# stardist/stardist

Hardware: AMD Instinct MI355X
Metric: predict_instances() Mpix/s (2D) + Mvox/s (3D) end-to-end at 1/2/4/8 GPU (higher is better)
Workload: dtype f32

## Files before the change

### include/stardist_hip.h

```cpp
#ifndef STARDIST_HIP_H
#define STARDIST_HIP_H

#include <stdbool.h>
#include <stdint.h>

#ifdef __cplusplus
extern "C" {
#endif

const char* sd_last_error(void);
int sd_version(void);
int sd_device_count(void);
int sd_release_workspace(void);
int sd_set_option(const char* name, int value);
int sd_get_option(const char* name);

int sd_nms2d_host(const float* dist, const float* points, int n_polys, int n_rays,
                  int use_kdtree, int use_bbox, int verbose, float threshold,
                  uint8_t* keep, int64_t* stats);
int sd_nms2d_device(const float* d_dist, const float* d_points, int n_polys, int n_rays,
                    int use_kdtree, int use_bbox, int verbose, float threshold,
                    uint8_t* d_keep, int64_t* stats, void* stream);

int sd_nms2d_old_host(const int32_t* polys, int n_polys, int n_rays, const int32_t* mapping, int height, int width,
                      float threshold, int max_bbox_search, int grid_y, int grid_x, int verbose, uint8_t* keep);
int sd_nms2d_old_device(const int32_t* d_polys, int n_polys, int n_rays, const int32_t* d_mapping, int height, int width,
                        float threshold, int max_bbox_search, int grid_y, int grid_x, int verbose, uint8_t* d_keep, void* stream);

int sd_prepare_polys_device(const int32_t* d_x, const int32_t* d_y, int n_polys, int n_verts, void* d_out,
                            int64_t out_bytes, void* stream);

int sd_clip_pairs_device(const int32_t* d_xa, const int32_t* d_ya, const int32_t* d_xb,
                         const int32_t* d_yb, int n_pairs, int n_verts,
                         int64_t* d_out_twice_area, int32_t* d_out_flags, void* stream);

int sd_area_bounds_pairs_device(const int32_t* d_xa, const int32_t* d_ya, const int32_t* d_xb, const int32_t* d_yb, int n_pairs,
                                int n_verts, float* d_out_area, float* d_out_band, int32_t* d_out_info, void* stream);

int sd_star_dist2d_host(const uint16_t* src, int H, int W, int n_rays, int grid_y, int grid_x,
                        float* dst);
int sd_star_dist2d_device(const uint16_t* d_src, int H, int W, int n_rays, int grid_y,
                          int grid_x, float* d_dst, void* stream);
int sd_star_dist3d_host(const uint16_t* src, int Z, int Y, int X, const float* dz,
                        const float* dy, const float* dx, int n_rays, int grid_z, int grid_y,
                        int grid_x, float* dst);
int sd_star_dist3d_device(const uint16_t* d_src, int Z, int Y, int X, const float* d_dz,
                          const float* d_dy, const float* d_dx, int n_rays, int grid_z,
                          int grid_y, int grid_x, float* d_dst, void* stream);

int sd_edt_prob_device(const int32_t* d_lbl, int Z, int Y, int X, double sz, double sy, double sx, int max_label,
                       float* d_prob, void* stream);

int sd_polygons_to_label_host(const float* coord, const int32_t* labels, int n_polys, int n_rays,
                              int H, int W, int32_t* result);
int sd_polygons_to_label_device(const float* d_coord, const int32_t* d_labels, int n_polys,
                                int n_rays, int H, int W, int32_t* d_result, void* stream);
int sd_polygons_to_label_window_device(const float* d_coord, const int32_t* d_labels, int n_polys, int n_rays, int HI, int WI,
                                       int y0, int x0, int H, int W, int32_t* d_result, void* stream);

int sd_dist_to_coord_device(const float* d_dist, const double* d_points, const double* d_sincos, long long n_polys, int n_rays,
// ... 157 lines not shown
```

### stardist_amd/csrc/area_bounds.h

```cpp
#pragma once
#include <hip/hip_runtime.h>

namespace sdarea {

enum { PP_PLAIN = 1, PP_POS = 2, PP_NEG = 4 };
struct PolyProps { float lmax, perim; int flags; int xmin, xmax, ymin, ymax; int pad; };

__device__ __forceinline__ float sgnf(float v) { return v > 0.f ? 1.f : (v < 0.f ? -1.f : 0.f); }
__device__ __forceinline__ float half_sum(float v) { for (int o = 16; o; o >>= 1) v += __shfl_xor(v, o); return v; }
__device__ __forceinline__ float half_max(float v) { for (int o = 16; o; o >>= 1) v = fmaxf(v, __shfl_xor(v, o)); return v; }
__device__ __forceinline__ int half_sum_i(int v) { for (int o = 16; o; o >>= 1) v += __shfl_xor(v, o); return v; }
__device__ __forceinline__ int half_min_i(int v) { for (int o = 16; o; o >>= 1) { const int t = __shfl_xor(v, o); v = t < v ? t : v; } return v; }
__device__ __forceinline__ int half_max_i(int v) { for (int o = 16; o; o >>= 1) { const int t = __shfl_xor(v, o); v = t > v ? t : v; } return v; }

constexpr float NEAR_W = 0.15f, STRIP_W = 0.45f;
constexpr int WINDOW = 2047;

static __global__ void __launch_bounds__(256) k_poly_props(const int* __restrict__ vx, const int* __restrict__ vy, int n, int R, PolyProps* __restrict__ out) {
  const int lane = threadIdx.x & 63, half = lane >> 5, l = lane & 31, hb = half << 5;
  const int wave = blockIdx.x * (blockDim.x >> 6) + (threadIdx.x >> 6);
  const int cand = 2 * wave + half;
  const bool cv = cand < n;
  const bool valid = cv && l < R;
  int X = 0, Y = 0;
  if (valid) { X = vx[(size_t)cand * R + l]; Y = vy[(size_t)cand * R + l]; }
  const int x0 = __shfl(X, hb), y0 = __shfl(Y, hb);
  const int xmin = half_min_i(valid ? X : 0x7fffffff), xmax = half_max_i(valid ? X : (int)0x80000000);
  const int ymin = half_min_i(valid ? Y : 0x7fffffff), ymax = half_max_i(valid ? Y : (int)0x80000000);
  const bool small = cv && (long long)xmax - xmin <= WINDOW && (long long)ymax - ymin <= WINDOW;
  const int ln = (l + 1 >= R) ? 0 : l + 1;
  const int rx = valid && small ? X - x0 : 0, ry = valid && small ? Y - y0 : 0;
  const int rbx = __shfl(rx, hb + ln), rby = __shfl(ry, hb + ln);
  const float ax = (float)rx, ay = (float)ry, bx = (float)rbx, by = (float)rby;
  const float ex = bx - ax, ey = by - ay;
  const bool deg = !valid || (ex == 0.f && ey == 0.f);
  const unsigned long long bal = __ballot(!deg);
  const unsigned int m32 = (unsigned int)(half ? (bal >> 32) : bal);
  const int count = __popc(m32);
  int nxt = -1;
  if (m32) { const unsigned int above = (l >= 31) ? 0u : (m32 & ~((2u << l) - 1u)); nxt = above ? __ffs((int)above) - 1 : __ffs((int)m32) - 1; }
  const int area2 = half_sum_i(valid ? rx * rby - ry * rbx : 0);
  bool bad = false;
  __shared__ float2 sv[4][2][32];
  __shared__ int sn[4][2][32];
  const int wv = threadIdx.x >> 6;
  sv[wv][half][l] = make_float2(ax, ay); sn[wv][half][l] = nxt;
  __builtin_amdgcn_wave_barrier();
  for (int dd = 1; dd <= (R >> 1); ++dd) {
    int k = l + dd; if (k >= R) k -= R;
    if (!valid) k = 0;
    const int kn = (k + 1 >= R) ? 0 : k + 1;
    const float2 c2 = sv[wv][half][k], d2 = sv[wv][half][kn];
    const float cx = c2.x, cy = c2.y, dx = d2.x, dy = d2.y;
    const int nxt_k = sn[wv][half][k];
    const bool degk = ((m32 >> k) & 1u) == 0u;
    const float fx = dx - cx, fy = dy - cy;
    if (valid && small && !degk && !((cx == ax && cy == ay) || (dx == ax && dy == ay)) && ay >= fminf(cy, dy) && ay <= fmaxf(cy, dy)) {
      if (fy == 0.f) { if (ax >= fminf(cx, dx) && ax <= fmaxf(cx, dx)) bad = true; }
      else if (2.f * fabsf((cx - ax) * fy + (ay - cy) * fx) <= fabsf(fy)) bad = true;
    }
    if (valid && small && !deg && !((ax == cx && ay == cy) || (bx == cx && by == cy)) && cy >= fminf(ay, by) && cy <= fmaxf(ay, by)) {
      if (ey == 0.f) { if (cx >= fminf(ax, bx) && cx <= fmaxf(ax, bx)) bad = true; }
      else if (2.f * fabsf((ax - cx) * ey + (cy - ay) * ex) <= fabsf(ey)) bad = true;
    }
    if (deg || degk || !valid) continue;
    if (k == nxt || nxt_k == l) {
      const float cr = ex * fy - ey * fx, dt = ex * fx + ey * fy;
      if (cr == 0.f && dt < 0.f) bad = true;
      continue;
    }
    const float o1 = ex * (cy - ay) - ey * (cx - ax), o2 = ex * (dy - ay) - ey * (dx - ax);
    const float o3 = fx * (ay - cy) - fy * (ax - cx), o4 = fx * (by - cy) - fy * (bx - cx);
    bool inter = (sgnf(o1) * sgnf(o2) <= 0.f) && (sgnf(o3) * sgnf(o4) <= 0.f);
    if (o1 == 0.f && o2 == 0.f)
      inter = fmaxf(fminf(ax, bx), fminf(cx, dx)) <= fminf(fmaxf(ax, bx), fmaxf(cx, dx)) &&
              fmaxf(fminf(ay, by), fminf(cy, dy)) <= fminf(fmaxf(ay, by), fmaxf(cy, dy));
    if (inter) bad = true;
  }
  const unsigned long long badm = __ballot(bad);
  const bool anybad = (unsigned int)(half ? (badm >> 32) : badm) != 0u;
  const float lmax = half_max(deg ? 0.f : sqrtf(ex * ex + ey * ey));
  const float perim = half_sum(deg ? 0.f : fabsf(ex) + fabsf(ey));
  if (cv && l == 0) {
    PolyProps p;
    p.lmax = lmax * (1.f + 1e-6f); p.perim = perim;
    p.flags = ((small && !anybad && count >= 3 && area2 != 0) ? PP_PLAIN : 0) | (area2 > 0 ? PP_POS : 0) | (area2 < 0 ? PP_NEG : 0);
    p.xmin = xmin; p.xmax = xmax; p.ymin = ymin; p.ymax = ymax; p.pad = 0;
    out[cand] = p;
  }
}

struct Enclosure { float area, band; int crossings, near; bool usable; };

__device__ __forceinline__ Enclosure pair_enclosure(const int* __restrict__ px, const int* __restrict__ py, const int* __restrict__ qx,
                                                    const int* __restrict__ qy, int R, const PolyProps& pp, const PolyProps& pq, bool active,
                                                    float2* sq, int l, int half) {
  Enclosure E; E.area = 0.f; E.band = 0.f; E.crossings = 0; E.near = 0; E.usable = false;
  const int hb = half << 5;
  bool use = active && (pp.flags & PP_PLAIN) && (pq.flags & PP_PLAIN) && ((pp.flags & (PP_POS | PP_NEG)) == (pq.flags & (PP_POS | PP_NEG)));
  const int ox = use ? (int)(((long long)pp.xmin + pp.xmax) >> 1) : 0, oy = use ? (int)(((long long)pp.ymin + pp.ymax) >> 1) : 0;
  long long ext = 0;
  if (use) {
    const long long e0 = (long long)pp.xmax - ox, e1 = (long long)ox - pp.xmin, e2 = (long long)pp.ymax - oy, e3 = (long long)oy - pp.ymin;
    const long long e4 = (long long)pq.xmax - ox, e5 = (long long)ox - pq.xmin, e6 = (long long)pq.ymax - oy, e7 = (long long)oy - pq.ymin;
    ext = e0; ext = e1 > ext ? e1 : ext; ext = e2 > ext ? e2 : ext; ext = e3 > ext ? e3 : ext;
    ext = e4 > ext ? e4 : ext; ext = e5 > ext ? e5 : ext; ext = e6 > ext ? e6 : ext; ext = e7 > ext ? e7 : ext;
    if (ext > WINDOW / 2) use = false;
  }
  const bool lv = use && l < R;
  float ax = 0.f, ay = 0.f, cqx = 0.f, cqy = 0.f;
  if (lv) { ax = (float)(px[l] - ox); ay = (float)(py[l] - oy); cqx = (float)(qx[l] - ox); cqy = (float)(qy[l] - oy); }
  sq[l] = make_float2(cqx, cqy);
  const int ln = (l + 1 >= R) ? 0 : l + 1;
// ... 83 lines not shown
```

### stardist_amd/csrc/area_bounds.hip

```cpp
#include "common.h"
#include "area_bounds.h"
#include "../../include/stardist_hip.h"

namespace {
__global__ void __launch_bounds__(256) k_area_probe(const int* __restrict__ xa, const int* __restrict__ ya, const int* __restrict__ xb,
                                                    const int* __restrict__ yb, int n, int R, const sdarea::PolyProps* __restrict__ pa,
                                                    const sdarea::PolyProps* __restrict__ pb, float* __restrict__ out_area, float* __restrict__ out_band,
                                                    int* __restrict__ out_info) {
  __shared__ float2 sq[4][2][32];
  const int lane = threadIdx.x & 63, half = lane >> 5, l = lane & 31, wv = threadIdx.x >> 6;
  const long long nw = (long long)gridDim.x * 4;
  for (long long base = 2ll * ((long long)blockIdx.x * 4 + wv); base < n; base += 2ll * nw) {
    const long long t = base + half;
    const bool active = t < n;
    const long long tt = active ? t : 0;
    const sdarea::Enclosure E = sdarea::pair_enclosure(xa + tt * R, ya + tt * R, xb + tt * R, yb + tt * R, R, pa[tt], pb[tt], active, sq[wv][half], l, half);
    if (active && l == 0) { out_area[t] = E.area; out_band[t] = E.band; out_info[t] = (E.usable ? 1 : 0) | ((E.crossings & 0x3FF) << 8) | ((E.near & 0x7FF) << 18); }
    __builtin_amdgcn_wave_barrier();
  }
}
}

extern "C" int sd_area_bounds_pairs_device(const int32_t* d_xa, const int32_t* d_ya, const int32_t* d_xb, const int32_t* d_yb, int n_pairs, int n_verts,
                                           float* d_out_area, float* d_out_band, int32_t* d_out_info, void* stream) {
  hipStream_t s = (hipStream_t)stream;
  if (n_pairs <= 0) return 0;
  const int R = n_verts;
  if (R < 3 || R > 32) { sd::set_error("sd_area_bounds_pairs: n_verts=%d unsupported (3..32)", R); return -1; }
  sd::Arena& A = sd::arena();
  if (A.begin(s)) return -1;
  sdarea::PolyProps* pa = (sdarea::PolyProps*)A.take((size_t)n_pairs * sizeof(sdarea::PolyProps));
  sdarea::PolyProps* pb = (sdarea::PolyProps*)A.take((size_t)n_pairs * sizeof(sdarea::PolyProps));
  if (!pa || !pb) return -1;
  hipLaunchKernelGGL(sdarea::k_poly_props, dim3(sd::div_up(n_pairs, 8)), dim3(256), 0, s, d_xa, d_ya, n_pairs, R, pa);
  hipLaunchKernelGGL(sdarea::k_poly_props, dim3(sd::div_up(n_pairs, 8)), dim3(256), 0, s, d_xb, d_yb, n_pairs, R, pb);
  const int blocks = sd::div_up(n_pairs, 8) < 2048 ? sd::div_up(n_pairs, 8) : 2048;
  hipLaunchKernelGGL(k_area_probe, dim3(blocks), dim3(256), 0, s, d_xa, d_ya, d_xb, d_yb, n_pairs, R, pa, pb, d_out_area, d_out_band, d_out_info);
  SD_LAUNCH_CHECK();
  SD_CHECK(hipStreamSynchronize(s));
  return 0;
}
```

### stardist_amd/csrc/nms2d.hip

```cpp
#include <type_traits>

#include "common.h"
#include "clip_sweep.h"
#include "clip_beam.h"
#include "area_bounds.h"
#include "../../include/stardist_hip.h"
#include <hipcub/hipcub.hpp>
#include <math.h>
#include <stdlib.h>
#include <vector>

namespace {

using sdclip::i64;

enum { ST_UNDECIDED = 0, ST_KEPT = 1, ST_SUPPRESSED = 2 };

__device__ __forceinline__ float wave_min(float v) { for (int o = 32; o; o >>= 1) v = fminf(v, __shfl_xor(v, o)); return v; }
__device__ __forceinline__ float wave_max(float v) { for (int o = 32; o; o >>= 1) v = fmaxf(v, __shfl_xor(v, o)); return v; }
__device__ __forceinline__ i64 wave_sum(i64 v) { for (int o = 32; o; o >>= 1) v += __shfl_xor(v, o); return v; }

__global__ void __launch_bounds__(256) k_build(const float* __restrict__ dist, const float* __restrict__ pts,
                                               const float2* __restrict__ sincos, int N, int R,
                                               int* __restrict__ vx, int* __restrict__ vy, int4* __restrict__ bbox,
                                               float* __restrict__ radius, float* __restrict__ area, int* gstats) {
  extern __shared__ int lds[];
  const int wave = threadIdx.x >> 6, lane = threadIdx.x & 63;
  const int i = blockIdx.x * (blockDim.x >> 6) + wave;
// ... 712 lines not shown
}

__global__ void k_count_after(unsigned int* out, const unsigned int* total, const unsigned int* first) { *out = *total > *first ? *total - *first : 0u; }
__global__ void k_iota(int* a, int n) { int i = blockIdx.x * blockDim.x + threadIdx.x; if (i < n) a[i] = i; }
__global__ void k_keep(const unsigned char* __restrict__ state, unsigned char* __restrict__ keep, int n) {
  int i = blockIdx.x * blockDim.x + threadIdx.x;
  if (i < n) keep[i] = (state[i] != ST_SUPPRESSED);
}

}

namespace sd {
int clip_full_pairs(const int2* d_pairs, const unsigned int* d_idx, const unsigned int* d_n, unsigned int cap, int R, const int* d_vx, const int* d_vy,
                    const float* d_area, float thr, unsigned char* d_state, unsigned char* d_supp, unsigned int* d_errCount, hipStream_t stream);
}

namespace {
struct Counters { int nU, nK, nS, left; unsigned long long nPairs; unsigned int nSpill, nExact, nErr, nDecided; };

template <int MAXV, int SPREP>
struct BeamPath {
  typedef sdclip::PolyPrep<MAXV> Prep;
  static int prepare(const int* vx, const int* vy, int N, int R, void* prep, hipStream_t s) {
    const size_t lds = sdclip::PrepWork<sdclip::LdsStorage<SPREP>, MAXV>::lds_bytes() + 64;
    hipLaunchKernelGGL((k_prepare<MAXV, SPREP>), dim3(sd::div_up(N, SPREP)), dim3(SPREP), lds, s, vx, vy, N, R, (Prep*)prep);
    SD_LAUNCH_CHECK();
    return 0;
  }
  static int tier1(const int2* pairs, const unsigned int* idx, const unsigned long long* nPairs, const unsigned int* first, const void* prep, const float* area,
                   float thr, unsigned char* state, unsigned char* supp, PairQueues q, hipStream_t s) {
    const int lanes = sd::option(sd::OPT_NMS2D_PAIR_LANES);
    if (lanes == 32) {
      static const size_t lds32 = beam_lds_bytes<MAXV, 8, 6, 4, 32>();
      hipLaunchKernelGGL((k_pairs_beam<MAXV, 8, 6, 4, 32, unsigned long long>), dim3(256 * 8), dim3(32), lds32, s, pairs, idx, nPairs, first, (const Prep*)prep, area, thr, state, supp, q);
    } else if (lanes == 6464) {
      static const size_t lds = beam_lds_bytes<MAXV, 8, 6, 4, 64>();
      hipLaunchKernelGGL((k_pairs_beam<MAXV, 8, 6, 4, 64, unsigned long long>), dim3(256 * 4), dim3(64), lds, s, pairs, idx, nPairs, first, (const Prep*)prep, area, thr, state, supp, q);
    } else {
      static const size_t lds16 = beam_lds_bytes<MAXV, 8, 6, 4, 64, true>();
      static const int per_cu = (int)((160 * 1024) / lds16);
      hipLaunchKernelGGL((k_pairs_beam<MAXV, 8, 6, 4, 64, unsigned long long, true>), dim3(256 * per_cu), dim3(64), lds16, s, pairs, idx, nPairs, first, (const Prep*)prep, area, thr, state, supp, q);
    }
    SD_LAUNCH_CHECK();
    return 0;
  }
  template <typename CNT>
  static int tier2(const int2* pairs, const unsigned int* idx, const CNT* nPairs, const unsigned int* first, const void* prep, const float* area, float thr,
                   unsigned char* state, unsigned char* supp, PairQueues q, hipStream_t s) {
    static const size_t lds = beam_lds_bytes<MAXV, 15, 16, 8, 32>();
    hipLaunchKernelGGL((k_pairs_beam<MAXV, 15, 16, 8, 32, CNT>), dim3(256 * 3), dim3(32), lds, s, pairs, idx, nPairs, first, (const Prep*)prep, area, thr, state, supp, q);
// ... 68 lines not shown
  if (R <= 32) prepStride = sizeof(sdclip::PolyPrep<32>); else if (R <= 64) prepStride = sizeof(sdclip::PolyPrep<64>);
  else if (R <= 128) prepStride = sizeof(sdclip::PolyPrep<128>); else prepStride = sizeof(sdclip::PolyPrep<256>);
  void* prep = A.take((size_t)N * prepStride);
  if (!prep) return -1;
  hipStream_t side = side_stream();
  if (!side) return -1;
  hipEvent_t evFork = nullptr, evJoin = nullptr;
  SD_CHECK(hipEventCreateWithFlags(&evFork, hipEventDisableTiming));
  SD_CHECK(hipEventCreateWithFlags(&evJoin, hipEventDisableTiming));
  EvGuard evguardFJ{evFork, evJoin};
  const bool areaBounds = R <= 32 && R >= 3 && sd::option(sd::OPT_NMS2D_AREA_BOUNDS) != 0 && sd::option(sd::OPT_NMS2D_STRICT) == 0;
  sdarea::PolyProps* props = nullptr;
  hipEvent_t evProps = nullptr, evPrep = nullptr;
  SD_CHECK(hipEventCreateWithFlags(&evProps, hipEventDisableTiming));
  SD_CHECK(hipEventCreateWithFlags(&evPrep, hipEventDisableTiming));
  EvGuard evguardP{evProps, evPrep};
  if (areaBounds) {
    props = (sdarea::PolyProps*)A.take((size_t)N * sizeof(sdarea::PolyProps));
    if (!props) return -1;
  }
  auto launch_side = [&]() -> int {
    SD_CHECK(hipEventRecord(evFork, s));
    SD_CHECK(hipStreamWaitEvent(side, evFork, 0));
    if (areaBounds) {
      hipLaunchKernelGGL(sdarea::k_poly_props, dim3(sd::div_up(N, 8)), dim3(256), 0, side, vx, vy, N, R, props);
      SD_LAUNCH_CHECK();
    }
    SD_CHECK(hipEventRecord(evProps, side));
    int rc;
    if (R <= 32) rc = BeamPath<32, 64>::prepare(vx, vy, N, R, prep, side);
    else if (R <= 64) rc = BeamPath<64, 64>::prepare(vx, vy, N, R, prep, side);
    else if (R <= 128) rc = BeamPath<128, 32>::prepare(vx, vy, N, R, prep, side);
    else rc = BeamPath<256, 16>::prepare(vx, vy, N, R, prep, side);
    if (rc) return -1;
    SD_CHECK(hipEventRecord(evPrep, side));
    SD_CHECK(hipEventRecord(evJoin, side));
    return 0;
  };
  int gs[8];
  SD_CHECK(hipMemcpyAsync(gs, gstats, sizeof(gs), hipMemcpyDeviceToHost, s));
  SD_CHECK(hipStreamSynchronize(s));
  float max_dist;
  memcpy(&max_dist, &gs[0], 4);

  GridP g;
  const float reach = (max_dist + 1.f) * 1.0001f + 1e-3f;
  const int by_bbox = (threshold >= 0.f || use_bbox) ? 1 : 0;
  float cs = 0.5f * reach;
  if (!(cs >= 1.f)) cs = 1.f;
  for (;;) {
    g.ny = (int)(((double)gs[2] - gs[1]) / cs) + 1;
    g.nx = (int)(((double)gs[4] - gs[3]) / cs) + 1;
    if ((long long)g.ny * g.nx <= (1ll << 26)) break;
    cs *= 2.f;
  }
  g.y0 = (float)gs[1]; g.x0 = (float)gs[3]; g.inv_cs = 1.f / cs;
  const int nCells = g.ny * g.nx;
// ... 501 lines not shown
```

### stardist_amd/csrc/nms2d_full.hip

```cpp
#include <type_traits>

#include "common.h"
#include "clip_sweep.h"
#include "clip_sweep_full.h"
#include "clip_beam.h"
#include <stdlib.h>
#include "../../include/stardist_hip.h"

namespace {
using sdclip::i64;

enum { ST_SUPPRESSED_ = 2 };
template <int MAXV, int MAXIL, int MAXREC, int MAXPT, int MAXJ>
__global__ void __launch_bounds__(64) k_full_pairs(const int2* __restrict__ pairs, const unsigned int* __restrict__ idx, const unsigned int* __restrict__ nPtr, unsigned int cap, int R,
                                                   const int* __restrict__ vx, const int* __restrict__ vy,
                                                   const float* __restrict__ area, float thr, unsigned char* __restrict__ state, unsigned char* __restrict__ supp,
                                                   unsigned int* errCount) {
  unsigned int n = *nPtr; if (n > cap) n = cap;
  for (unsigned int t = threadIdx.x * gridDim.x + blockIdx.x; t < n; t += gridDim.x * blockDim.x) {
    if (MAXV > 64 && __hip_atomic_load(errCount, __ATOMIC_RELAXED, __HIP_MEMORY_SCOPE_AGENT) != 0u) break;
    const unsigned int p = idx ? idx[t] : t;
    const int2 ij = pairs[p];
    sdclip::SweepFull<MAXV, MAXIL, MAXREC, MAXPT, MAXJ> sw;
    sw.reset_state();
    sw.add_path(vx + (size_t)ij.x * R, vy + (size_t)ij.x * R, R, sdclip::kClip, 0);
    sw.add_path(vx + (size_t)ij.y * R, vy + (size_t)ij.y * R, R, sdclip::kSubject, MAXV);
    const i64 twice = sw.execute();
    if (sw.status & ~sdclip::ST_FAIL) atomicAdd(errCount, 1u);
// ... 107 lines not shown
  if (R <= 32) {
    static const size_t ldsBytes = lds_full_bytes<32, 64, 32, 192, 64>();
    static bool attr_set = false;
    if (!attr_set) {
      SD_CHECK(hipFuncSetAttribute((const void*)k_full_pairs_lds<32, 64, 32, 192, 64>, hipFuncAttributeMaxDynamicSharedMemorySize, (int)ldsBytes));
      attr_set = true;
    }
    hipLaunchKernelGGL((k_full_pairs_lds<32, 64, 32, 192, 64>), dim3(1024), dim3(LDSF_T), ldsBytes, s, d_pairs, d_idx, d_n, cap, R, d_vx, d_vy, d_area, thr, d_state, d_supp, d_errCount);
  } else if (R <= 64) hipLaunchKernelGGL((k_full_pairs<64, 96, 48, 384, 96>), dim3(2048), dim3(64), 0, s, d_pairs, d_idx, d_n, cap, R, d_vx, d_vy, d_area, thr, d_state, d_supp, d_errCount);
  else if (R <= 128) hipLaunchKernelGGL((k_full_pairs<128, 128, 64, 768, 128>), dim3(512), dim3(64), 0, s, d_pairs, d_idx, d_n, cap, R, d_vx, d_vy, d_area, thr, d_state, d_supp, d_errCount);
  else hipLaunchKernelGGL((k_full_pairs<256, 192, 96, 1536, 192>), dim3(256), dim3(64), 0, s, d_pairs, d_idx, d_n, cap, R, d_vx, d_vy, d_area, thr, d_state, d_supp, d_errCount);
  SD_LAUNCH_CHECK();
  return 0;
}
}

extern "C" int sd_prepare_polys_device(const int32_t* d_x, const int32_t* d_y, int n_polys, int n_verts, void* d_out, int64_t out_bytes, void* stream) {
  hipStream_t s = (hipStream_t)stream;
  const int R = n_verts;
  if (n_polys <= 0) return 0;
  if (R < 1 || R > 256) { sd::set_error("sd_prepare_polys: n_verts=%d unsupported (1..256)", R); return -1; }
  const size_t rec = R <= 32 ? sizeof(sdclip::PolyPrep<32>) : R <= 64 ? sizeof(sdclip::PolyPrep<64>) : R <= 128 ? sizeof(sdclip::PolyPrep<128>) : sizeof(sdclip::PolyPrep<256>);
  if ((int64_t)(rec * (size_t)n_polys) > out_bytes) { sd::set_error("sd_prepare_polys: output buffer too small (%zu bytes per polygon)", rec); return -1; }
  if (R <= 32) return launch_prepare_probe<32, 64>(d_x, d_y, n_polys, R, d_out, s);
  if (R <= 64) return launch_prepare_probe<64, 64>(d_x, d_y, n_polys, R, d_out, s);
  if (R <= 128) return launch_prepare_probe<128, 32>(d_x, d_y, n_polys, R, d_out, s);
  return launch_prepare_probe<256, 16>(d_x, d_y, n_polys, R, d_out, s);
}

extern "C" int sd_clip_pairs_device(const int32_t* d_xa, const int32_t* d_ya, const int32_t* d_xb, const int32_t* d_yb,
                                    int n_pairs, int n_verts, int64_t* d_out_twice_area, int32_t* d_out_flags,
                                    void* stream) {
  hipStream_t s = (hipStream_t)stream;
  if (n_pairs <= 0) return 0;
  const int R = n_verts;
  if (R < 1 || R > 256) { sd::set_error("sd_clip_pairs: n_verts=%d unsupported (1..256)", R); return -1; }
  i64* out = (i64*)d_out_twice_area;
  const int tier = sd::option(sd::OPT_PROBE_TIER);
  if (R <= 32 && tier == 1) return launch_probe<32, 8, 6, 4, 64, 64, 32, 192, 64, true>(d_xa, d_ya, d_xb, d_yb, n_pairs, R, out, d_out_flags, s);
  if (R <= 32 && tier == 3) return launch_probe<32, 8, 6, 4, 64, 64, 32, 192, 64>(d_xa, d_ya, d_xb, d_yb, n_pairs, R, out, d_out_flags, s);
  if (R <= 32) return launch_probe<32, 15, 16, 8, 32, 64, 32, 192, 64>(d_xa, d_ya, d_xb, d_yb, n_pairs, R, out, d_out_flags, s);
  if (R <= 64) return launch_probe<64, 15, 16, 8, 32, 96, 48, 384, 96>(d_xa, d_ya, d_xb, d_yb, n_pairs, R, out, d_out_flags, s);
  if (R <= 128) return launch_probe<128, 15, 16, 8, 32, 128, 64, 768, 128>(d_xa, d_ya, d_xb, d_yb, n_pairs, R, out, d_out_flags, s);
  return launch_probe<256, 15, 16, 8, 16, 192, 96, 1536, 192>(d_xa, d_ya, d_xb, d_yb, n_pairs, R, out, d_out_flags, s);
}
```

### stardist_amd/lib/_native.py

```python
import ctypes
import os

import numpy as np

_HERE = os.path.dirname(os.path.abspath(__file__))
LIB_PATH = os.path.join(_HERE, "..", "csrc", "libstardist_hip.so")

_lib = None
last_stats = {}

_c_f32p = ctypes.POINTER(ctypes.c_float)
_c_i32p = ctypes.POINTER(ctypes.c_int32)
_c_i64p = ctypes.POINTER(ctypes.c_int64)
_c_u8p = ctypes.POINTER(ctypes.c_uint8)
_c_u16p = ctypes.POINTER(ctypes.c_uint16)
_vp = ctypes.c_void_p
_i = ctypes.c_int
_f = ctypes.c_float

SIGNATURES = {
    "sd_last_error": (ctypes.c_char_p, []),
    "sd_version": (_i, []),
    "sd_device_count": (_i, []),
    "sd_release_workspace": (_i, []),
    "sd_set_option": (_i, [ctypes.c_char_p, _i]),
    "sd_get_option": (_i, [ctypes.c_char_p]),
    "sd_nms2d_host": (_i, [_vp, _vp, _i, _i, _i, _i, _i, _f, _vp, _vp]),
    "sd_nms2d_device": (_i, [_vp, _vp, _i, _i, _i, _i, _i, _f, _vp, _vp, _vp]),
    "sd_nms2d_old_host": (_i, [_vp, _i, _i, _vp, _i, _i, _f, _i, _i, _i, _i, _vp]),
    "sd_nms2d_old_device": (_i, [_vp, _i, _i, _vp, _i, _i, _f, _i, _i, _i, _i, _vp, _vp]),
    "sd_clip_pairs_device": (_i, [_vp, _vp, _vp, _vp, _i, _i, _vp, _vp, _vp]),
    "sd_area_bounds_pairs_device": (_i, [_vp, _vp, _vp, _vp, _i, _i, _vp, _vp, _vp, _vp]),
    "sd_prepare_polys_device": (_i, [_vp, _vp, _i, _i, _vp, ctypes.c_int64, _vp]),
    "sd_star_dist2d_host": (_i, [_vp, _i, _i, _i, _i, _i, _vp]),
    "sd_star_dist2d_device": (_i, [_vp, _i, _i, _i, _i, _i, _vp, _vp]),
    "sd_star_dist3d_host": (_i, [_vp, _i, _i, _i, _vp, _vp, _vp, _i, _i, _i, _i, _vp]),
    "sd_star_dist3d_device": (_i, [_vp, _i, _i, _i, _vp, _vp, _vp, _i, _i, _i, _i, _vp, _vp]),
    "sd_edt_prob_device": (_i, [_vp, _i, _i, _i, ctypes.c_double, ctypes.c_double, ctypes.c_double, _i, _vp, _vp]),
    "sd_dist_to_coord_device": (_i, [_vp, _vp, _vp, ctypes.c_longlong, _i, ctypes.c_double, ctypes.c_double, _vp, _vp]),
    "sd_polygons_to_label_host": (_i, [_vp, _vp, _i, _i, _i, _i, _vp]),
    "sd_polygons_to_label_device": (_i, [_vp, _vp, _i, _i, _i, _i, _vp, _vp]),
    "sd_polygons_to_label_window_device": (_i, [_vp, _vp, _i, _i, _i, _i, _i, _i, _i, _i, _vp, _vp]),
    "sd_polyhedron_to_label_window_device": (_i, [_vp, _vp, _vp, _vp, _i, _i, _i, _vp] + [_i] * 13 + [_vp, _vp]),
    "_LIB_non_maximum_suppression_sparse": (None, [_vp, _vp, _vp, _i, _i, _i, _vp, _vp, _f, _i, _i, _i, _vp]),
    "sd_nms3d_device": (_i, [_vp, _vp, _vp, _i, _i, _i, _vp, _vp, _f, _i, _i, _i, _vp, _vp, _vp]),
    "sd_hiv_pairs_device": (_i, [_vp, _vp, _i, _i, _i, _vp, _vp, _vp, _i, _vp, _vp, _vp]),
    "_LIB_polyhedron_to_label": (None, [_vp, _vp, _vp, _vp, _i, _i, _i, _vp, _i, _i, _i, _i, _i, _i, _i, _vp]),
    "sd_polyhedron_to_label_device": (_i, [_vp, _vp, _vp, _vp, _i, _i, _i, _vp, _i, _i, _i, _i, _i, _i, _i, _vp, _vp]),
    "sd_select_candidates_device": (_i, [_vp, _vp, _i, _vp, _vp, _i, _f, _i, _vp, _vp, _vp, _vp, _vp]),
    "sd_survivor_positions_device": (_i, [_vp, ctypes.c_longlong, _vp, _vp, _vp]),
    "sd_survivors2d_device": (_i, [_vp, _i, _vp, _vp, _vp, _i, _vp, _vp, _vp, _vp, _vp, _vp, _vp]),
    "sd_sorted_rows_device": (_i, [_vp, _vp, _i, _i, _vp, _vp, _vp, _vp, _vp, _vp, _vp]),
    "sd_sort_scores_desc_device": (_i, [_vp, _i, _vp, _vp, _vp]),
    "sd_bias_act_device": (_i, [_vp, _vp, ctypes.c_longlong, _i, ctypes.c_longlong, _i, _vp]),
    "sd_add_bias_act_device": (_i, [_vp, _vp, _vp, ctypes.c_longlong, _i, ctypes.c_longlong, _i, _vp]),
    "sd_maxpool_ndhwc_device": (_i, [_vp, _i, _i, _i, _i, _i, _i, _i, _vp, _vp]),
# ... 127 lines not shown
```

Before: 299.9.

## Fuse polygon property and clip-prep passes into one per-polygon kernel

Replaces the separate polygon-properties kernel and the clip preparation kernel for polygons with up to 32 vertices with a single kernel that loads each polygon's vertices once and computes both outputs. The preparation step gets a fast path that packs vertices as 16-bit relative coordinates in a shared-memory ring, and the self-intersection test skips edge pairs whose bounding boxes cannot touch, using a wave-wide vote. This is meant to cut one launch and one global read of the vertices, and to reduce the per-polygon work in the NMS setup. In exchange the kernel is more complex, uses one 64-thread block per 64 polygons, and runs the props and prep work one after the other instead of overlapping them.

```diff
diff --git a/include/stardist_hip.h b/include/stardist_hip.h
--- a/include/stardist_hip.h
+++ b/include/stardist_hip.h
@@ -36,6 +36,8 @@
 
 int sd_area_bounds_pairs_device(const int32_t* d_xa, const int32_t* d_ya, const int32_t* d_xb, const int32_t* d_yb, int n_pairs,
                                 int n_verts, float* d_out_area, float* d_out_band, int32_t* d_out_info, void* stream);
+
+int sd_poly_pass_device(const int32_t* d_x, const int32_t* d_y, int n_polys, int n_verts, void* d_props, void* d_prep, void* stream);
 
 int sd_star_dist2d_host(const uint16_t* src, int H, int W, int n_rays, int grid_y, int grid_x,
                         float* dst);
diff --git a/stardist_amd/csrc/area_bounds.h b/stardist_amd/csrc/area_bounds.h
--- a/stardist_amd/csrc/area_bounds.h
+++ b/stardist_amd/csrc/area_bounds.h
@@ -16,79 +16,6 @@
 constexpr float NEAR_W = 0.15f, STRIP_W = 0.45f;
 constexpr int WINDOW = 2047;
 
-static __global__ void __launch_bounds__(256) k_poly_props(const int* __restrict__ vx, const int* __restrict__ vy, int n, int R, PolyProps* __restrict__ out) {
-  const int lane = threadIdx.x & 63, half = lane >> 5, l = lane & 31, hb = half << 5;
-  const int wave = blockIdx.x * (blockDim.x >> 6) + (threadIdx.x >> 6);
-  const int cand = 2 * wave + half;
-  const bool cv = cand < n;
-  const bool valid = cv && l < R;
-  int X = 0, Y = 0;
-  if (valid) { X = vx[(size_t)cand * R + l]; Y = vy[(size_t)cand * R + l]; }
-  const int x0 = __shfl(X, hb), y0 = __shfl(Y, hb);
-  const int xmin = half_min_i(valid ? X : 0x7fffffff), xmax = half_max_i(valid ? X : (int)0x80000000);
-  const int ymin = half_min_i(valid ? Y : 0x7fffffff), ymax = half_max_i(valid ? Y : (int)0x80000000);
-  const bool small = cv && (long long)xmax - xmin <= WINDOW && (long long)ymax - ymin <= WINDOW;
-  const int ln = (l + 1 >= R) ? 0 : l + 1;
-  const int rx = valid && small ? X - x0 : 0, ry = valid && small ? Y - y0 : 0;
-  const int rbx = __shfl(rx, hb + ln), rby = __shfl(ry, hb + ln);
-  const float ax = (float)rx, ay = (float)ry, bx = (float)rbx, by = (float)rby;
-  const float ex = bx - ax, ey = by - ay;
-  const bool deg = !valid || (ex == 0.f && ey == 0.f);
-  const unsigned long long bal = __ballot(!deg);
-  const unsigned int m32 = (unsigned int)(half ? (bal >> 32) : bal);
-  const int count = __popc(m32);
-  int nxt = -1;
-  if (m32) { const unsigned int above = (l >= 31) ? 0u : (m32 & ~((2u << l) - 1u)); nxt = above ? __ffs((int)above) - 1 : __ffs((int)m32) - 1; }
-  const int area2 = half_sum_i(valid ? rx * rby - ry * rbx : 0);
-  bool bad = false;
-  __shared__ float2 sv[4][2][32];
-  __shared__ int sn[4][2][32];
-  const int wv = threadIdx.x >> 6;
-  sv[wv][half][l] = make_float2(ax, ay); sn[wv][half][l] = nxt;
-  __builtin_amdgcn_wave_barrier();
-  for (int dd = 1; dd <= (R >> 1); ++dd) {
-    int k = l + dd; if (k >= R) k -= R;
-    if (!valid) k = 0;
-    const int kn = (k + 1 >= R) ? 0 : k + 1;
-    const float2 c2 = sv[wv][half][k], d2 = sv[wv][half][kn];
-    const float cx = c2.x, cy = c2.y, dx = d2.x, dy = d2.y;
-    const int nxt_k = sn[wv][half][k];
-    const bool degk = ((m32 >> k) & 1u) == 0u;
-    const float fx = dx - cx, fy = dy - cy;
-    if (valid && small && !degk && !((cx == ax && cy == ay) || (dx == ax && dy == ay)) && ay >= fminf(cy, dy) && ay <= fmaxf(cy, dy)) {
-      if (fy == 0.f) { if (ax >= fminf(cx, dx) && ax <= fmaxf(cx, dx)) bad = true; }
-      else if (2.f * fabsf((cx - ax) * fy + (ay - cy) * fx) <= fabsf(fy)) bad = true;
-    }
-    if (valid && small && !deg && !((ax == cx && ay == cy) || (bx == cx && by == cy)) && cy >= fminf(ay, by) && cy <= fmaxf(ay, by)) {
-      if (ey == 0.f) { if (cx >= fminf(ax, bx) && cx <= fmaxf(ax, bx)) bad = true; }
-      else if (2.f * fabsf((ax - cx) * ey + (cy - ay) * ex) <= fabsf(ey)) bad = true;
-    }
-    if (deg || degk || !valid) continue;
-    if (k == nxt || nxt_k == l) {
-      const float cr = ex * fy - ey * fx, dt = ex * fx + ey * fy;
-      if (cr == 0.f && dt < 0.f) bad = true;
-      continue;
-    }
-    const float o1 = ex * (cy - ay) - ey * (cx - ax), o2 = ex * (dy - ay) - ey * (dx - ax);
-    const float o3 = fx * (ay - cy) - fy * (ax - cx), o4 = fx * (by - cy) - fy * (bx - cx);
-    bool inter = (sgnf(o1) * sgnf(o2) <= 0.f) && (sgnf(o3) * sgnf(o4) <= 0.f);
-    if (o1 == 0.f && o2 == 0.f)
-      inter = fmaxf(fminf(ax, bx), fminf(cx, dx)) <= fminf(fmaxf(ax, bx), fmaxf(cx, dx)) &&
-              fmaxf(fminf(ay, by), fminf(cy, dy)) <= fminf(fmaxf(ay, by), fmaxf(cy, dy));
-    if (inter) bad = true;
-  }
-  const unsigned long long badm = __ballot(bad);
-  const bool anybad = (unsigned int)(half ? (badm >> 32) : badm) != 0u;
-  const float lmax = half_max(deg ? 0.f : sqrtf(ex * ex + ey * ey));
-  const float perim = half_sum(deg ? 0.f : fabsf(ex) + fabsf(ey));
-  if (cv && l == 0) {
-    PolyProps p;
-    p.lmax = lmax * (1.f + 1e-6f); p.perim = perim;
-    p.flags = ((small && !anybad && count >= 3 && area2 != 0) ? PP_PLAIN : 0) | (area2 > 0 ? PP_POS : 0) | (area2 < 0 ? PP_NEG : 0);
-    p.xmin = xmin; p.xmax = xmax; p.ymin = ymin; p.ymax = ymax; p.pad = 0;
-    out[cand] = p;
-  }
-}
 
 struct Enclosure { float area, band; int crossings, near; bool usable; };
 
diff --git a/stardist_amd/csrc/area_bounds.hip b/stardist_amd/csrc/area_bounds.hip
--- a/stardist_amd/csrc/area_bounds.hip
+++ b/stardist_amd/csrc/area_bounds.hip
@@ -1,5 +1,6 @@
 #include "common.h"
 #include "area_bounds.h"
+#include "poly_pass.h"
 #include "../../include/stardist_hip.h"
 
 namespace {
@@ -32,11 +33,23 @@
   sdarea::PolyProps* pa = (sdarea::PolyProps*)A.take((size_t)n_pairs * sizeof(sdarea::PolyProps));
   sdarea::PolyProps* pb = (sdarea::PolyProps*)A.take((size_t)n_pairs * sizeof(sdarea::PolyProps));
   if (!pa || !pb) return -1;
-  hipLaunchKernelGGL(sdarea::k_poly_props, dim3(sd::div_up(n_pairs, 8)), dim3(256), 0, s, d_xa, d_ya, n_pairs, R, pa);
-  hipLaunchKernelGGL(sdarea::k_poly_props, dim3(sd::div_up(n_pairs, 8)), dim3(256), 0, s, d_xb, d_yb, n_pairs, R, pb);
+  if (sdpass::launch_poly_pass(d_xa, d_ya, n_pairs, R, pa, nullptr, s) || sdpass::launch_poly_pass(d_xb, d_yb, n_pairs, R, pb, nullptr, s)) {
+    sd::set_error("sd_area_bounds_pairs: launch failed");
+    return -1;
+  }
   const int blocks = sd::div_up(n_pairs, 8) < 2048 ? sd::div_up(n_pairs, 8) : 2048;
   hipLaunchKernelGGL(k_area_probe, dim3(blocks), dim3(256), 0, s, d_xa, d_ya, d_xb, d_yb, n_pairs, R, pa, pb, d_out_area, d_out_band, d_out_info);
   SD_LAUNCH_CHECK();
   SD_CHECK(hipStreamSynchronize(s));
   return 0;
 }
+
+extern "C" int sd_poly_pass_device(const int32_t* d_x, const int32_t* d_y, int n_polys, int n_verts, void* d_props, void* d_prep, void* stream) {
+  hipStream_t s = (hipStream_t)stream;
+  if (n_polys <= 0 || (!d_props && !d_prep)) return 0;
+  const int R = n_verts;
+  if (R < (d_props ? 3 : 1) || R > 32) { sd::set_error("sd_poly_pass: n_verts=%d unsupported (%d..32)", R, d_props ? 3 : 1); return -1; }
+  if (sdpass::launch_poly_pass(d_x, d_y, n_polys, R, (sdarea::PolyProps*)d_props, d_prep, s)) { sd::set_error("sd_poly_pass: launch failed"); return -1; }
+  SD_CHECK(hipStreamSynchronize(s));
+  return 0;
+}
diff --git a/stardist_amd/csrc/nms2d.hip b/stardist_amd/csrc/nms2d.hip
--- a/stardist_amd/csrc/nms2d.hip
+++ b/stardist_amd/csrc/nms2d.hip
@@ -4,6 +4,7 @@
 #include "clip_sweep.h"
 #include "clip_beam.h"
 #include "area_bounds.h"
+#include "poly_pass.h"
 #include "../../include/stardist_hip.h"
 #include <hipcub/hipcub.hpp>
 #include <math.h>
@@ -762,10 +763,15 @@
 struct BeamPath {
   typedef sdclip::PolyPrep<MAXV> Prep;
   static int prepare(const int* vx, const int* vy, int N, int R, void* prep, hipStream_t s) {
-    const size_t lds = sdclip::PrepWork<sdclip::LdsStorage<SPREP>, MAXV>::lds_bytes() + 64;
-    hipLaunchKernelGGL((k_prepare<MAXV, SPREP>), dim3(sd::div_up(N, SPREP)), dim3(SPREP), lds, s, vx, vy, N, R, (Prep*)prep);
-    SD_LAUNCH_CHECK();
-    return 0;
+    if constexpr (MAXV == 32) {
+      if (sdpass::launch_poly_pass(vx, vy, N, R, nullptr, prep, s)) { sd::set_error("sd_nms2d: launch of the per-polygon pass failed"); return -1; }
+      return 0;
+    } else {
+      const size_t lds = sdclip::PrepWork<sdclip::LdsStorage<SPREP>, MAXV>::lds_bytes() + 64;
+      hipLaunchKernelGGL((k_prepare<MAXV, SPREP>), dim3(sd::div_up(N, SPREP)), dim3(SPREP), lds, s, vx, vy, N, R, (Prep*)prep);
+      SD_LAUNCH_CHECK();
+      return 0;
+    }
   }
   static int tier1(const int2* pairs, const unsigned int* idx, const unsigned long long* nPairs, const unsigned int* first, const void* prep, const float* area,
                    float thr, unsigned char* state, unsigned char* supp, PairQueues q, hipStream_t s) {
@@ -880,17 +886,13 @@
   auto launch_side = [&]() -> int {
     SD_CHECK(hipEventRecord(evFork, s));
     SD_CHECK(hipStreamWaitEvent(side, evFork, 0));
-    if (areaBounds) {
-      hipLaunchKernelGGL(sdarea::k_poly_props, dim3(sd::div_up(N, 8)), dim3(256), 0, side, vx, vy, N, R, props);
-      SD_LAUNCH_CHECK();
-    }
-    SD_CHECK(hipEventRecord(evProps, side));
     int rc;
-    if (R <= 32) rc = BeamPath<32, 64>::prepare(vx, vy, N, R, prep, side);
+    if (R <= 32) rc = sdpass::launch_poly_pass(vx, vy, N, R, props, prep, side);
     else if (R <= 64) rc = BeamPath<64, 64>::prepare(vx, vy, N, R, prep, side);
     else if (R <= 128) rc = BeamPath<128, 32>::prepare(vx, vy, N, R, prep, side);
     else rc = BeamPath<256, 16>::prepare(vx, vy, N, R, prep, side);
-    if (rc) return -1;
+    if (rc) { sd::set_error("sd_nms2d: launch of the per-polygon pass failed"); return -1; }
+    SD_CHECK(hipEventRecord(evProps, side));
     SD_CHECK(hipEventRecord(evPrep, side));
     SD_CHECK(hipEventRecord(evJoin, side));
     return 0;
diff --git a/stardist_amd/csrc/nms2d_full.hip b/stardist_amd/csrc/nms2d_full.hip
--- a/stardist_amd/csrc/nms2d_full.hip
+++ b/stardist_amd/csrc/nms2d_full.hip
@@ -4,6 +4,7 @@
 #include "clip_sweep.h"
 #include "clip_sweep_full.h"
 #include "clip_beam.h"
+#include "poly_pass.h"
 #include <stdlib.h>
 #include "../../include/stardist_hip.h"
 
@@ -157,7 +158,10 @@
   if (R < 1 || R > 256) { sd::set_error("sd_prepare_polys: n_verts=%d unsupported (1..256)", R); return -1; }
   const size_t rec = R <= 32 ? sizeof(sdclip::PolyPrep<32>) : R <= 64 ? sizeof(sdclip::PolyPrep<64>) : R <= 128 ? sizeof(sdclip::PolyPrep<128>) : sizeof(sdclip::PolyPrep<256>);
   if ((int64_t)(rec * (size_t)n_polys) > out_bytes) { sd::set_error("sd_prepare_polys: output buffer too small (%zu bytes per polygon)", rec); return -1; }
-  if (R <= 32) return launch_prepare_probe<32, 64>(d_x, d_y, n_polys, R, d_out, s);
+  if (R <= 32) {
+    if (sdpass::launch_poly_pass(d_x, d_y, n_polys, R, nullptr, d_out, s)) { sd::set_error("sd_prepare_polys: launch failed"); return -1; }
+    return 0;
+  }
   if (R <= 64) return launch_prepare_probe<64, 64>(d_x, d_y, n_polys, R, d_out, s);
   if (R <= 128) return launch_prepare_probe<128, 32>(d_x, d_y, n_polys, R, d_out, s);
   return launch_prepare_probe<256, 16>(d_x, d_y, n_polys, R, d_out, s);
diff --git a/stardist_amd/csrc/poly_pass.h b/stardist_amd/csrc/poly_pass.h
--- /dev/null
+++ b/stardist_amd/csrc/poly_pass.h
@@ -0,0 +1,365 @@
+#pragma once
+#include "clip_sweep.h"
+#include "clip_beam.h"
+
+namespace sdpass {
+
+typedef long long i64;
+constexpr int PASS_T = 64;
+constexpr int PASS_V = 32;
+
+SD_HD int px_(int p) { return (int)(short)(p & 0xffff); }
+SD_HD int py_(int p) { return p >> 16; }
+SD_HD int pack_(int x, int y) { return (int)(((unsigned)y << 16) | ((unsigned)x & 0xffffu)); }
+
+struct FastPrep {
+  const int* ring;
+  int n;
+  unsigned swm, l1m, l2m;
+
+  SD_HD int P(int i) const { return ring[i * PASS_T]; }
+  SD_HD int cx(int i) const { return px_(P(i)); }
+  SD_HD int cy(int i) const { return py_(P(i)); }
+  SD_HD int nx(int e) const { return e + 1 == n ? 0 : e + 1; }
+  SD_HD int pv(int e) const { return e == 0 ? n - 1 : e - 1; }
+  SD_HD bool sw(int e) const { return (swm >> e) & 1u; }
+  SD_HD int lmlc(int e) const { return ((l1m >> e) & 1u) ? 1 : (((l2m >> e) & 1u) ? 2 : 0); }
+  SD_HD int botx(int e) const { return sw(e) ? cx(nx(e)) : cx(e); }
+  SD_HD int boty(int e) const { return sw(e) ? cy(nx(e)) : cy(e); }
+  SD_HD int topx(int e) const { return sw(e) ? cx(e) : cx(nx(e)); }
+  SD_HD int topy(int e) const { return sw(e) ? cy(e) : cy(nx(e)); }
+  SD_HD bool is_horz(int e) const { return cy(e) == cy(nx(e)); }
+  SD_HD double dx(int e) const {
+    const i64 dy = (i64)topy(e) - boty(e);
+    if (dy == 0) return SD_HORIZONTAL;
+    return (double)((i64)topx(e) - botx(e)) / (double)dy;
+  }
+  SD_HD void reverse_horizontal(int e) { swm ^= 1u << e; }
+  SD_HD void set_lml(int e, int c) {
+    const unsigned b = 1u << e;
+    l1m = (l1m & ~b) | (c == 1 ? b : 0u); l2m = (l2m & ~b) | (c == 2 ? b : 0u);
+  }
+
+  SD_HD int find_next_loc_min(int E) const {
+    bool done = false;
+    int guard = 0;
+    while (!done) {
+      while (botx(E) != botx(pv(E)) || boty(E) != boty(pv(E)) || (cx(E) == topx(E) && cy(E) == topy(E))) E = nx(E);
+      if (!is_horz(E) && !is_horz(pv(E))) done = true;
+      else {
+        while (is_horz(pv(E))) E = pv(E);
+        const int E2 = E;
+        while (is_horz(E)) E = nx(E);
+        if (topy(E) != boty(pv(E))) {
+          if (botx(pv(E2)) < botx(E)) E = E2;
+          done = true;
+        }
+      }
+      if (++guard > 4 * PASS_V) done = true;
+    }
+    return E;
+  }
+  SD_HD int process_bound(int E, bool fwd) {
+    int Result = E, Horz;
+    if (is_horz(E)) {
+      int EStart = fwd ? pv(E) : nx(E);
+      if (is_horz(EStart)) {
+        if (botx(EStart) != botx(E) && topx(EStart) != botx(E)) reverse_horizontal(E);
+      } else if (botx(EStart) != botx(E)) reverse_horizontal(E);
+    }
+    int EStart = E;
+    if (fwd) {
+      while (topy(Result) == boty(nx(Result))) Result = nx(Result);
+      if (is_horz(Result)) {
+        Horz = Result;
+        while (is_horz(pv(Horz))) Horz = pv(Horz);
+        if (topx(pv(Horz)) > topx(nx(Result))) Result = pv(Horz);
+      }
+      while (E != Result) {
+        set_lml(E, 1);
+        if (is_horz(E) && E != EStart && botx(E) != topx(pv(E))) reverse_horizontal(E);
+        E = nx(E);
+      }
+      if (is_horz(E) && E != EStart && botx(E) != topx(pv(E))) reverse_horizontal(E);
+      Result = nx(Result);
+    } else {
+      while (topy(Result) == boty(pv(Result))) Result = pv(Result);
+      if (is_horz(Result)) {
+        Horz = Result;
+        while (is_horz(nx(Horz))) Horz = nx(Horz);
+        if (topx(nx(Horz)) == topx(pv(Result)) || topx(nx(Horz)) > topx(pv(Result))) Result = nx(Horz);
+      }
+      while (E != Result) {
+        set_lml(E, 2);
+        if (is_horz(E) && E != EStart && botx(E) != topx(nx(E))) reverse_horizontal(E);
+        E = pv(E);
+      }
+      if (is_horz(E) && E != EStart && botx(E) != topx(nx(E))) reverse_horizontal(E);
+      Result = pv(Result);
+    }
+    return Result;
+  }
+
+  SD_HD void prepare(int* wring, int n_in, int ox, int oy, sdclip::PolyPrep<PASS_V>* out) {
+    typedef sdclip::PolyPrep<PASS_V> Prep;
+    ring = wring; n = 0; swm = l1m = l2m = 0u;
+    int m = 0, n_lm = 0, st = 0;
+    int highI = n_in - 1;
+    const int p0 = P(0);
+    while (highI > 0 && P(highI) == p0) --highI;
+    while (highI > 0 && P(highI) == P(highI - 1)) --highI;
+    if (highI >= 2) {
+      unsigned am = (highI >= 31) ? 0xffffffffu : ((2u << highI) - 1u);
+      auto nxt = [&](int e) { const unsigned above = am & ~((2u << e) - 1u); return above ? __builtin_ctz(above) : __builtin_ctz(am); };
+      auto prv = [&](int e) { const unsigned below = am & ((1u << e) - 1u); return below ? 31 - __builtin_clz(below) : 31 - __builtin_clz(am); };
+      int eStart = 0, E = 0, eLoopStop = 0;
+      for (;;) {
+        const int en = nxt(E);
+        const int pe = P(E), pn = P(en);
+        if (pe == pn) {
+          if (E == en) break;
+          if (E == eStart) eStart = en;
+          am &= ~(1u << E); E = en;
+          eLoopStop = E;
+          continue;
+        }
+        const int ep0 = prv(E);
+        if (ep0 == en) break;
+        const int pp = P(ep0);
+        if (((i64)py_(pp) - py_(pe)) * ((i64)px_(pe) - px_(pn)) == ((i64)px_(pp) - px_(pe)) * ((i64)py_(pe) - py_(pn))) {
+          if (E == eStart) eStart = en;
+          am &= ~(1u << E);
+          E = ep0;
+          eLoopStop = E;
+          continue;
+        }
+        E = en;
+        if (E == eLoopStop) break;
+      }
+      if (prv(E) != nxt(E)) {
+        const int E0 = __builtin_popcount(am & ((1u << eStart) - 1u));
+        for (int i = 0; i <= highI; ++i) {
+          if (!((am >> i) & 1u)) continue;
+          if (m != i) wring[m * PASS_T] = P(i);
+          ++m;
+        }
+        n = m;
+        bool isFlat = true;
+        const int y0c = cy(0);
+        for (int e = 0; e < m; ++e) {
+          const int en = nx(e);
+          const int ye = cy(e), yn = cy(en);
+          if (!(ye >= yn)) swm |= 1u << e;
+          if (yn != y0c) isFlat = false;
+        }
+        if (isFlat) m = 0;
+        else {
+          E = E0;
+          if (botx(pv(E)) == topx(pv(E)) && boty(pv(E)) == topy(pv(E))) E = nx(E);
+          int EMin = -1, guard = 0;
+          int lmy[sdclip::BEAM_MAXLM], lml[sdclip::BEAM_MAXLM], lmr[sdclip::BEAM_MAXLM];
+#pragma unroll
+          for (int i = 0; i < sdclip::BEAM_MAXLM; ++i) { lmy[i] = 0; lml[i] = 0; lmr[i] = 0; }
+          for (;;) {
+            E = find_next_loc_min(E);
+            if (E == EMin) break;
+            else if (EMin < 0) EMin = E;
+            if (++guard > 2 * PASS_V + 2) { st |= sdclip::ST_ITER; break; }
+            int left, right; bool leftFwd;
+            if (dx(E) < dx(pv(E))) { left = pv(E); right = E; leftFwd = false; }
+            else { left = E; right = pv(E); leftFwd = true; }
+            const int y = boty(E);
+            E = process_bound(left, leftFwd);
+            const int E2 = process_bound(right, !leftFwd);
+            if (n_lm < sdclip::BEAM_MAXLM) {
+              int k = 0;
+#pragma unroll
+              for (int i = 0; i < sdclip::BEAM_MAXLM; ++i) k += (i < n_lm && lmy[i] >= y) ? 1 : 0;
+#pragma unroll
+              for (int i = sdclip::BEAM_MAXLM - 1; i > 0; --i)
+                if (i > k && i <= n_lm) { lmy[i] = lmy[i - 1]; lml[i] = lml[i - 1]; lmr[i] = lmr[i - 1]; }
+#pragma unroll
+              for (int i = 0; i < sdclip::BEAM_MAXLM; ++i)
+                if (i == k) { lmy[i] = y; lml[i] = left; lmr[i] = right; }
+              ++n_lm;
+            } else st |= sdclip::ST_OVERFLOW_LM;
+            if (!leftFwd) E = E2;
+          }
+          for (int i = 0; i < m; ++i) { const int p = P(i); out->v[i].x = px_(p) + ox; out->v[i].y = py_(p) + oy; }
+          out->v[m].x = cx(0) + ox; out->v[m].y = cy(0) + oy;
+          for (int i = 0; i < m; ++i) {
+            const int c = lmlc(i);
+            const int nl = (c == 1) ? nx(i) : (c == 2 ? pv(i) : -1);
+            int cc = c | (sw(i) ? 4 : 0);
+            if (nl >= 0 && is_horz(nl)) cc |= 8;
+            out->ecode[i] = (unsigned char)cc;
+            const int a = nx(i), b = pv(i);
+            int mp = Prep::NONE;
+            if (topx(a) == topx(i) && topy(a) == topy(i) && lmlc(a) == 0) mp = a;
+            else if (topx(b) == topx(i) && topy(b) == topy(i) && lmlc(b) == 0) mp = b;
+            out->mpair[i] = (typename Prep::pidx)mp;
+            int last = i, g2 = 0;
+            if (is_horz(i)) {
+              for (;;) {
+                const int c2 = lmlc(last);
+                const int n2 = (c2 == 1) ? nx(last) : (c2 == 2 ? pv(last) : -1);
+                if (n2 < 0 || !is_horz(n2)) break;
+                last = n2;
+                if (++g2 > PASS_V) { st |= sdclip::ST_ITER; break; }
+              }
+            }
+            out->hlast[i] = (typename Prep::pidx)last;
+          }
+#pragma unroll
+          for (int i = 0; i < sdclip::BEAM_MAXLM; ++i)
+            if (i < n_lm) { out->lm_left[i] = (typename Prep::pidx)lml[i]; out->lm_right[i] = (typename Prep::pidx)lmr[i]; }
+        }
+      } else m = 0;
+    }
+    if (m == 0) { n_lm = 0; st = 0; }
+    out->n = m; out->n_lm = n_lm; out->status = st; out->pad = 0;
+  }
+};
+
+}
+
+#if defined(__HIPCC__)
+#include <hip/hip_runtime.h>
+#include "area_bounds.h"
+
+namespace sdpass {
+
+__device__ __forceinline__ sdarea::PolyProps props_pair(int X, int Y, bool cv, bool valid, int R, int l, int half, float2* sv) {
+  using namespace sdarea;
+  const int hb = half << 5;
+  const int x0 = __shfl(X, hb), y0 = __shfl(Y, hb);
+  const int xmin = half_min_i(valid ? X : 0x7fffffff), xmax = half_max_i(valid ? X : (int)0x80000000);
+  const int ymin = half_min_i(valid ? Y : 0x7fffffff), ymax = half_max_i(valid ? Y : (int)0x80000000);
+  const bool small = cv && (long long)xmax - xmin <= WINDOW && (long long)ymax - ymin <= WINDOW;
+  const int ln = (l + 1 >= R) ? 0 : l + 1;
+  const int rx = valid && small ? X - x0 : 0, ry = valid && small ? Y - y0 : 0;
+  const int rbx = __shfl(rx, hb + ln), rby = __shfl(ry, hb + ln);
+  const float ax = (float)rx, ay = (float)ry, bx = (float)rbx, by = (float)rby;
+  const float ex = bx - ax, ey = by - ay;
+  const bool deg = !valid || (ex == 0.f && ey == 0.f);
+  const unsigned long long bal = __ballot(!deg);
+  const unsigned int m32 = (unsigned int)(half ? (bal >> 32) : bal);
+  const int count = __popc(m32);
+  auto next_of = [&](int e) {
+    int r = -1;
+    if (m32) { const unsigned int above = (e >= 31) ? 0u : (m32 & ~((2u << e) - 1u)); r = above ? __ffs((int)above) - 1 : __ffs((int)m32) - 1; }
+    return r;
+  };
+  const int nxt = next_of(l);
+  const int area2 = half_sum_i(valid ? rx * rby - ry * rbx : 0);
+  bool bad = false;
+  __builtin_amdgcn_fence(__ATOMIC_RELEASE, "wavefront");
+  __builtin_amdgcn_wave_barrier();
+  sv[l] = make_float2(ax, ay);
+  __builtin_amdgcn_wave_barrier();
+  const float exlo = fminf(ax, bx) - 1.f, exhi = fmaxf(ax, bx) + 1.f, eylo = fminf(ay, by) - 1.f, eyhi = fmaxf(ay, by) + 1.f;
+  for (int dd = 1; dd <= (R >> 1); ++dd) {
+    int k = l + dd; if (k >= R) k -= R;
+    if (!valid) k = 0;
+    const int kn = (k + 1 >= R) ? 0 : k + 1;
+    const float2 c2 = sv[k], d2 = sv[kn];
+    const float cx = c2.x, cy = c2.y, dx = d2.x, dy = d2.y;
+    const int nxt_k = next_of(k);
+    const bool degk = ((m32 >> k) & 1u) == 0u;
+    const bool boxes = (fminf(cx, dx) <= exhi) & (fmaxf(cx, dx) >= exlo) & (fminf(cy, dy) <= eyhi) & (fmaxf(cy, dy) >= eylo);
+    if (!__any(valid && small && (boxes || k == nxt || nxt_k == l))) continue;
+    const float fx = dx - cx, fy = dy - cy;
+    if (valid && small && !degk && !((cx == ax && cy == ay) || (dx == ax && dy == ay)) && ay >= fminf(cy, dy) && ay <= fmaxf(cy, dy)) {
+      if (fy == 0.f) { if (ax >= fminf(cx, dx) && ax <= fmaxf(cx, dx)) bad = true; }
+      else if (2.f * fabsf((cx - ax) * fy + (ay - cy) * fx) <= fabsf(fy)) bad = true;
+    }
+    if (valid && small && !deg && !((ax == cx && ay == cy) || (bx == cx && by == cy)) && cy >= fminf(ay, by) && cy <= fmaxf(ay, by)) {
+      if (ey == 0.f) { if (cx >= fminf(ax, bx) && cx <= fmaxf(ax, bx)) bad = true; }
+      else if (2.f * fabsf((ax - cx) * ey + (cy - ay) * ex) <= fabsf(ey)) bad = true;
+    }
+    if (deg || degk || !valid) continue;
+    if (k == nxt || nxt_k == l) {
+      const float cr = ex * fy - ey * fx, dt = ex * fx + ey * fy;
+      if (cr == 0.f && dt < 0.f) bad = true;
+      continue;
+    }
+    const float o1 = ex * (cy - ay) - ey * (cx - ax), o2 = ex * (dy - ay) - ey * (dx - ax);
+    const float o3 = fx * (ay - cy) - fy * (ax - cx), o4 = fx * (by - cy) - fy * (bx - cx);
+    bool inter = (sgnf(o1) * sgnf(o2) <= 0.f) && (sgnf(o3) * sgnf(o4) <= 0.f);
+    if (o1 == 0.f && o2 == 0.f)
+      inter = fmaxf(fminf(ax, bx), fminf(cx, dx)) <= fminf(fmaxf(ax, bx), fmaxf(cx, dx)) &&
+              fmaxf(fminf(ay, by), fminf(cy, dy)) <= fminf(fmaxf(ay, by), fmaxf(cy, dy));
+    if (inter) bad = true;
+  }
+  const unsigned long long badm = __ballot(bad);
+  const bool anybad = (unsigned int)(half ? (badm >> 32) : badm) != 0u;
+  const float lmax = half_max(deg ? 0.f : sqrtf(ex * ex + ey * ey));
+  const float perim = half_sum(deg ? 0.f : fabsf(ex) + fabsf(ey));
+  PolyProps p;
+  p.lmax = lmax * (1.f + 1e-6f); p.perim = perim;
+  p.flags = ((small && !anybad && count >= 3 && area2 != 0) ? PP_PLAIN : 0) | (area2 > 0 ? PP_POS : 0) | (area2 < 0 ? PP_NEG : 0);
+  p.xmin = xmin; p.xmax = xmax; p.ymin = ymin; p.ymax = ymax; p.pad = 0;
+  return p;
+}
+
+template <bool PROPS, bool PREP>
+__global__ void __launch_bounds__(PASS_T) k_poly_pass(const int* __restrict__ vx, const int* __restrict__ vy, int n, int R,
+                                                      sdarea::PolyProps* __restrict__ props, sdclip::PolyPrep<PASS_V>* __restrict__ prep) {
+  __shared__ int ring[PREP ? PASS_V * PASS_T : 1];
+  __shared__ float2 sv[2][32];
+  const int lane = threadIdx.x, half = lane >> 5, l = lane & 31;
+  const int base = blockIdx.x * PASS_T;
+  int myx0 = 0, myy0 = 0;
+  unsigned long long fitm = 0;
+  for (int p = 0; p < PASS_T / 2; ++p) {
+    const int t = 2 * p + half;
+    if (base + 2 * p >= n) break;
+    const int cand = base + t;
+    const bool cv = cand < n;
+    const bool valid = cv && l < R;
+    int X = 0, Y = 0;
+    if (valid) { X = vx[(size_t)cand * R + l]; Y = vy[(size_t)cand * R + l]; }
+    if (PROPS) {
+      const sdarea::PolyProps pr = props_pair(X, Y, cv, valid, R, l, half, sv[half]);
+      if (cv && l == 0) props[cand] = pr;
+    }
+    if (PREP) {
+      const int x0 = __shfl(X, half << 5), y0 = __shfl(Y, half << 5);
+      const long long rx = (long long)X - x0, ry = (long long)Y - y0;
+      const bool fits = rx >= -32768 && rx <= 32767 && ry >= -32768 && ry <= 32767;
+      const unsigned long long nf = __ballot(valid && !fits);
+      const bool hfit = cv && (unsigned int)(half ? (nf >> 32) : nf) == 0u;
+      if (valid && hfit) ring[l * PASS_T + t] = pack_((int)rx, (int)ry);
+      const unsigned long long fb = __ballot(hfit && l == 0);
+      fitm |= ((fb & 1ull) << (2 * p)) | (((fb >> 32) & 1ull) << (2 * p + 1));
+      const int x00 = __builtin_amdgcn_readlane(X, 0), y00 = __builtin_amdgcn_readlane(Y, 0);
+      const int x01 = __builtin_amdgcn_readlane(X, 32), y01 = __builtin_amdgcn_readlane(Y, 32);
+      if (lane == 2 * p) { myx0 = x00; myy0 = y00; }
+      if (lane == 2 * p + 1) { myx0 = x01; myy0 = y01; }
+    }
+  }
+  if (!PREP) return;
+  __syncthreads();
+  const int cand = base + lane;
+  if (cand >= n) return;
+  if ((fitm >> lane) & 1ull) {
+    FastPrep w;
+    w.prepare(ring + lane, R, myx0, myy0, prep + cand);
+  } else {
+    sdclip::PrepWork<sdclip::PlainStorage, PASS_V> w;
+    w.prepare(vx + (size_t)cand * R, vy + (size_t)cand * R, R, prep + cand);
+  }
+}
+
+inline int launch_poly_pass(const int* vx, const int* vy, int n, int R, sdarea::PolyProps* props, void* prep, hipStream_t s) {
+  if (n <= 0 || (!props && !prep)) return 0;
+  const dim3 grid((n + PASS_T - 1) / PASS_T), block(PASS_T);
+  typedef sdclip::PolyPrep<PASS_V> Prep;
+  if (props && prep) hipLaunchKernelGGL((k_poly_pass<true, true>), grid, block, 0, s, vx, vy, n, R, props, (Prep*)prep);
+  else if (props) hipLaunchKernelGGL((k_poly_pass<true, false>), grid, block, 0, s, vx, vy, n, R, props, (Prep*)nullptr);
+  else hipLaunchKernelGGL((k_poly_pass<false, true>), grid, block, 0, s, vx, vy, n, R, (sdarea::PolyProps*)nullptr, (Prep*)prep);
+  return hipGetLastError() == hipSuccess ? 0 : -1;
+}
+
+}
+#endif
diff --git a/stardist_amd/lib/_native.py b/stardist_amd/lib/_native.py
--- a/stardist_amd/lib/_native.py
+++ b/stardist_amd/lib/_native.py
@@ -32,6 +32,7 @@
     "sd_clip_pairs_device": (_i, [_vp, _vp, _vp, _vp, _i, _i, _vp, _vp, _vp]),
     "sd_area_bounds_pairs_device": (_i, [_vp, _vp, _vp, _vp, _i, _i, _vp, _vp, _vp, _vp]),
     "sd_prepare_polys_device": (_i, [_vp, _vp, _i, _i, _vp, ctypes.c_int64, _vp]),
+    "sd_poly_pass_device": (_i, [_vp, _vp, _i, _i, _vp, _vp, _vp]),
     "sd_star_dist2d_host": (_i, [_vp, _i, _i, _i, _i, _i, _vp]),
     "sd_star_dist2d_device": (_i, [_vp, _i, _i, _i, _i, _i, _vp, _vp]),
     "sd_star_dist3d_host": (_i, [_vp, _i, _i, _i, _vp, _vp, _vp, _i, _i, _i, _i, _vp]),
```

New measurement: 312.2 (median of 6 runs). 4.1% higher.
